# vkit-x/vkit

Measured on AMD Instinct MI355X. Metric: Mpixels/s (2048^2 RGB, geo+photo chain), higher is better.
Workload: dtype u8; 1 GPU; C3 fused chain: camera_cubic_curve remap (level 5) + gaussian_blur(sigma=1.0) + color_shift(37) + gaussion_noise(std=10.0, the numpy stream default_rng(5000 + i) drawn on the device inside every step), states built from the configs inside every step, 2048x2048x3 uint8, batch 256 per GPU; batch_per_gpu=256, image=2048x2048x3, noise_mode=tiles, states=built on the device from the configs inside every step (vkx_camera_states_dev), lanes=1

## Files before the change

### vkit_amd/csrc/fused.hip

```cpp
#include "vkx_internal.h"
#include "vkx_cell.h"
#include "vkx_color.h"

#include <float.h>
#include <memory>
#include <stdlib.h>
#include <string.h>

namespace {

constexpr int W = 64;
constexpr int RMAX = 3;
constexpr int NLDSCELL = 64;
#ifndef VKX_FUSED_NWAVES
#define VKX_FUSED_NWAVES 8
#endif
constexpr int NWAVES = VKX_FUSED_NWAVES;
constexpr int NTHREADS = 64 * NWAVES;
constexpr int ROWS_PER_WAVE = 8;
constexpr int WH = NWAVES * ROWS_PER_WAVE;
__host__ __device__ constexpr int tile_side(int R) { return (W - 2 * R) & ~3; }
__host__ __device__ constexpr int tile_height(int R) { return WH == W ? tile_side(R) : WH - 2 * R; }
#ifndef VKX_FUSED_CGROUP
#define VKX_FUSED_CGROUP 2
// ... 46 lines not shown
    int n;
};

struct TileRect {
    int x0, y0, x1, y1;
    __host__ __device__ bool empty() const { return x1 < x0 || y1 < y0; }
};
__host__ __device__ inline TileRect interior_rect(int dw, int dh, int R)
{
    const int Tw = tile_side(R), Th = tile_height(R);
    TileRect r;
    r.x0 = (R + Tw - 1) / Tw;
    r.y0 = (R + Th - 1) / Th;
    r.x1 = dw - W + R >= 0 ? (dw - W + R) / Tw : -1;
    r.y1 = dh - WH + R >= 0 ? (dh - WH + R) / Th : -1;
    return r;
}

struct TileBin {
    int rmin, cmin;
    int rmax1, cmax1;
};

struct CellR {
    int ex[4], edx[4];
    short vx[4], vy[4];
    int flags, pad;
};
static_assert(sizeof(CellR) == 56, "CellR mirrors the tail of CellC");

__device__ __forceinline__ int find_item(const int *__restrict__ prefix, int n, int v)
{
    int lo = 0, hi = n - 1;
    while (lo < hi) {
        const int mid = (lo + hi + 1) >> 1;
        if (prefix[mid] <= v) lo = mid; else hi = mid - 1;
    }
    return lo;
}

constexpr int kLocalBins = 1024;

__global__ void __launch_bounds__(256) k_chain_setup(const ItemDev *__restrict__ items, const int *__restrict__ cell_prefix,
                                                     int n_items, int total_cells, int slots,
                                                     vkc::CellC *__restrict__ cells, TileBin *__restrict__ bins,
                                                     int *__restrict__ deferred )
{
    __shared__ int lbins[kLocalBins * 4];
    __shared__ int s_item, s_tiles_x, s_ty_min, s_ty_max;
    const int gid = blockIdx.x * 256 + threadIdx.x;
    const bool active = gid < total_cells;
    int ii = -1, r = 0, c = 0, tx0 = 0, tx1 = -1, ty0 = 0, ty1 = -1, tiles_x = 1;
    if (active) {
        ii = find_item(cell_prefix, n_items, gid);
        const ItemDev &it = items[ii];
        const int cell = gid - it.cell_base;
        vkc::CellC rec;
        int xmin, xmax, ymin, ymax;
        if (vkc::build_cell<vkc::kCellDirectOnly>(it.sv, it.dv, it.rows, it.cols, cell, rec, xmin, xmax, ymin, ymax)) cells[gid] = rec;
        else deferred[1 + atomicAdd(&deferred[0], 1)] = gid;
        r = cell / (it.cols - 1); c = cell - r * (it.cols - 1);
        const int Tw = tile_side(it.R), Th = tile_height(it.R);
        tx0 = (xmin - it.R) / Tw; tx1 = (xmax + it.R) / Tw; ty0 = (ymin - it.R) / Th; ty1 = (ymax + it.R) / Th;
        if (xmin - it.R < 0) tx0 = 0;
        if (ymin - it.R < 0) ty0 = 0;
        tiles_x = it.tiles_x;
        tx1 = min(tx1, tiles_x - 1);
        ty1 = min(ty1, it.tiles_y - 1);
    }
    if (threadIdx.x == 0) { s_item = ii; s_tiles_x = tiles_x; s_ty_min = INT_MAX; s_ty_max = -1; }
    __syncthreads();
    const bool local = active && ii == s_item && ty0 <= ty1 && tx0 <= tx1;
    if (local) { atomicMin(&s_ty_min, ty0); atomicMax(&s_ty_max, ty1); }
    __syncthreads();
    const int tymin = s_ty_min, nb = s_ty_max >= tymin ? (s_ty_max - tymin + 1) * s_tiles_x : 0;
    const bool use_lds = nb > 0 && nb <= kLocalBins;
    if (use_lds)
        for (int i = threadIdx.x; i < nb; i += 256) {
            lbins[4 * i] = 0x7f7f7f7f; lbins[4 * i + 1] = 0x7f7f7f7f; lbins[4 * i + 2] = 0; lbins[4 * i + 3] = 0;
        }
    __syncthreads();
    for (int ty = ty0; ty <= ty1; ty++)
        for (int tx = tx0; tx <= tx1; tx++) {
            if (local && use_lds) {
                int *b = lbins + 4 * ((ty - tymin) * tiles_x + tx);
                atomicMin(b, r); atomicMin(b + 1, c); atomicMax(b + 2, r + 1); atomicMax(b + 3, c + 1);
            } else {
                TileBin *b = bins + (size_t)ii * slots + ty * tiles_x + tx;
                atomicMin(&b->rmin, r);
                atomicMin(&b->cmin, c);
                atomicMax(&b->rmax1, r + 1);
                atomicMax(&b->cmax1, c + 1);
            }
        }
    __syncthreads();
    if (use_lds)
        for (int i = threadIdx.x; i < nb; i += 256) {
            if (lbins[4 * i + 2] == 0) continue;
            TileBin *b = bins + (size_t)s_item * slots + tymin * s_tiles_x + i;
            atomicMin(&b->rmin, lbins[4 * i]);
            atomicMin(&b->cmin, lbins[4 * i + 1]);
            atomicMax(&b->rmax1, lbins[4 * i + 2]);
            atomicMax(&b->cmax1, lbins[4 * i + 3]);
        }
}

__global__ void __launch_bounds__(64) k_chain_setup_svd(const ItemDev *__restrict__ items, const int *__restrict__ cell_prefix,
                                                        int n_items, vkc::CellC *__restrict__ cells,
                                                        const int *__restrict__ deferred)
{
    const int n = deferred[0];
    const int sub = threadIdx.x & 7;
    for (int j = blockIdx.x * 8 + (threadIdx.x >> 3); j < n; j += gridDim.x * 8) {
        const int gid = deferred[1 + j];
        const ItemDev &it = items[find_item(cell_prefix, n_items, gid)];
        vkc::CellC rec;
        int xmin, xmax, ymin, ymax;
        vkc::build_cell<vkc::kCellJacobiGroup8>(it.sv, it.dv, it.rows, it.cols, gid - it.cell_base, rec, xmin, xmax, ymin, ymax);
        if (sub == 0) cells[gid] = rec;
    }
}

__device__ __forceinline__ int div_small(int n, int d, float rcp_d)
{
    int q = (int)(((float)n + 0.5f) * rcp_d);
    const int r = n - q * d;
    q += r >= d ? 1 : 0;
    q -= r < 0 ? 1 : 0;
    return q;
}

__device__ __forceinline__ uint32_t mad_u24(uint32_t a, uint32_t b, uint32_t c)
{
    uint32_t r;
    asm("v_mad_u32_u24 %0, %1, %2, %3" : "=v"(r) : "v"(a), "v"(b), "v"(c));
    return r;
}

__device__ __forceinline__ uint32_t mad_u24_ks(uint32_t k_uniform, uint32_t b, uint32_t c)
{
    return __umul24(k_uniform, b) + c;
}
__device__ __forceinline__ uint32_t mad_u24_cs(uint32_t a, uint32_t b, uint32_t c_uniform)
{
    return __umul24(a, b) + c_uniform;
}

typedef unsigned short ushort2_t __attribute__((ext_vector_type(2)));
__device__ __forceinline__ uint32_t dot2_u16_ks(uint32_t k_uniform, uint32_t b, uint32_t c)
{
    return __builtin_amdgcn_udot2(__builtin_bit_cast(ushort2_t, k_uniform), __builtin_bit_cast(ushort2_t, b), c, false);
}

__device__ __forceinline__ uint64_t uniform64(uint64_t v)
{
    const uint32_t lo = __builtin_amdgcn_readfirstlane((uint32_t)v), hi = __builtin_amdgcn_readfirstlane((uint32_t)(v >> 32));
    return ((uint64_t)hi << 32) | lo;
}

__device__ __forceinline__ void div_pair(double nx, double ny, double de, double &qx, double &qy)
{
    bool fdx, fdy, fnx, fny;
    const double sdx = __builtin_amdgcn_div_scale(nx, de, false, &fdx);
    const double sdy = __builtin_amdgcn_div_scale(ny, de, false, &fdy);
    if (__builtin_amdgcn_ballot_w64(__double_as_longlong(sdx) != __double_as_longlong(sdy)) != 0) {
        qx = nx / de;
        qy = ny / de;
        return;
    }
    double r = __builtin_amdgcn_rcp(sdx);
    double e = fma(-sdx, r, 1.0);
    r = fma(r, e, r);
    e = fma(-sdx, r, 1.0);
    r = fma(r, e, r);
    const double snx = __builtin_amdgcn_div_scale(nx, de, true, &fnx);
    const double sny = __builtin_amdgcn_div_scale(ny, de, true, &fny);
    const double px = snx * r, py = sny * r;
    const double ex = fma(-sdx, px, snx), ey = fma(-sdx, py, sny);
    qx = __builtin_amdgcn_div_fixup(__builtin_amdgcn_div_fmas(ex, r, px, fnx), de, nx);
    qy = __builtin_amdgcn_div_fixup(__builtin_amdgcn_div_fmas(ey, r, py, fny), de, ny);
}

__device__ __forceinline__ bool div_pair_f32_fast(double nx, double ny, double de, float &fx, float &fy)
{
    double r = __builtin_amdgcn_rcp(de);
    double e = fma(-de, r, 1.0);
    r = fma(r, e, r);
    e = fma(-de, r, 1.0);
    r = fma(r, e, r);
    const double qx = nx * r, qy = ny * r;
    const uint32_t lx = (uint32_t)__double_as_longlong(qx) & 0x1fffffffu, ly = (uint32_t)__double_as_longlong(qy) & 0x1fffffffu;
    const bool danger = (lx - (0x10000000u - 16u)) < 32u || (ly - (0x10000000u - 16u)) < 32u;
    fx = (float)qx;
    fy = (float)qy;
    return __builtin_amdgcn_ballot_w64(danger) == 0;
}

__device__ __forceinline__ void rim_sample_rgb(gsrc_t src, int sh, int sw, ptrdiff_t sstride, int X, int Y, uint32_t &prb, uint32_t &pg)
{
    const int sx = vkd::sat_short(X >> 5), sy = vkd::sat_short(Y >> 5);
    const int fx = X & 31, fy = Y & 31;
    prb = 0; pg = 0;
    if (sx >= sw || sx + 1 < 0 || sy >= sh || sy + 1 < 0) return;
    const bool x0 = sx >= 0, x1 = sx + 1 < sw, y0 = sy >= 0, y1 = sy + 1 < sh;
    const gsrc_t r0 = src + (ptrdiff_t)sy * sstride + (ptrdiff_t)sx * 3, r1 = r0 + sstride;
    const int w00 = (32 - fy) * (32 - fx), w01 = (32 - fy) * fx, w10 = fy * (32 - fx), w11 = fy * fx;
    uint32_t c[3];
#pragma unroll
    for (int k = 0; k < 3; k++) {
        const int v0 = (x0 && y0) ? r0[k] : 0;
        const int v1 = (x1 && y0) ? r0[3 + k] : 0;
        const int v2 = (x0 && y1) ? r1[k] : 0;
        const int v3 = (x1 && y1) ? r1[3 + k] : 0;
        c[k] = (uint32_t)(v0 * w00 + v1 * w01 + v2 * w10 + v3 * w11 + 512) >> 10;
    }
    prb = c[0] | (c[2] << 16);
    pg = c[1];
}

struct HsvLut {
    int sdiv[256];
    int hdiv[256];
};

__device__ __forceinline__ void hue_shift_px(const int *sdiv, const int *hdiv, int delta, int &r, int &g, int &b)
{
    int H, S, V;
    vkd::rgb2hsv_full<true>(sdiv, hdiv, r, g, b, H, S, V);
    H = (H + delta) & 255;
    vkd::hsv2rgb_full(H, S, V, r, g, b);
}

constexpr int P_ = 97;
constexpr int kPairPitch = 2 * P_;
constexpr size_t kLdsOwn = sizeof(uint32_t) * WH * P_;
constexpr size_t kLdsHbB = 1024;
constexpr size_t kLdsCellR = sizeof(CellR) * NLDSCELL;
constexpr size_t kLdsCellH = sizeof(double) * 9 * NLDSCELL;
constexpr size_t kLdsLut = sizeof(int) * 512;
constexpr size_t kLdsSel = sizeof(uint32_t) * 8;
constexpr size_t kLdsNoiseRows = sizeof(uint32_t) * 2 * WH;
constexpr size_t kFusedLds = kLdsOwn + kLdsHbB + kLdsCellR + kLdsCellH + kLdsLut + kLdsSel + 16 + kLdsNoiseRows;

typedef const double __attribute__((address_space(3))) *lds_cdouble_t;


__device__ __forceinline__ int cvt_i32_sat(float v)
{
    int r;
    asm("v_cvt_i32_f32 %0, %1" : "=v"(r) : "v"(v));
    return r;
}

__device__ __forceinline__ uint32_t add_noise_u8x4(uint32_t px, uint32_t n01, uint32_t n23)
{
    typedef unsigned short pk16 __attribute__((ext_vector_type(2)));
    pk16 lo = __builtin_bit_cast(pk16, __builtin_amdgcn_perm(px, px, 0x0c010c00u));
    pk16 hi = __builtin_bit_cast(pk16, __builtin_amdgcn_perm(px, px, 0x0c030c02u));
    lo += __builtin_bit_cast(pk16, n01);
    hi += __builtin_bit_cast(pk16, n23);
    uint32_t lo8, hi8;
    asm("v_sat_pk_u8_i16 %0, %1" : "=v"(lo8) : "v"(__builtin_bit_cast(uint32_t, lo)));
    asm("v_sat_pk_u8_i16 %0, %1" : "=v"(hi8) : "v"(__builtin_bit_cast(uint32_t, hi)));
    return __builtin_amdgcn_perm(hi8, lo8, 0x05040100u);
}

template <int KIND, bool STREAK = false, int RC = -1>
__device__ __forceinline__ void chain_tile(const ItemDev &it, const int tx, const int ty,
                                           const vkc::CellC *__restrict__ cells, const TileBin &bin,
                                           const HsvLut *__restrict__ lut, int phase_limit, const ElemPack *els = nullptr)
{
    constexpr bool INTERIOR = KIND == 1, EMPTY = KIND == 2;
    extern __shared__ __attribute__((aligned(16))) unsigned char smem[];
    uint32_t *own = (uint32_t *)smem;
    uint16_t *hbB = (uint16_t *)(smem + kLdsOwn);
    CellR *lcr = (CellR *)(smem + kLdsOwn + kLdsHbB);
    double *lch = (double *)(smem + kLdsOwn + kLdsHbB + kLdsCellR);
    int *lsdiv = (int *)(smem + kLdsOwn + kLdsHbB + kLdsCellR + kLdsCellH);
    int *lhdiv = lsdiv + 256;
    uint32_t *lsel = (uint32_t *)(lhdiv + 256);
    int *lflag = (int *)(lsel + 8);
    uint32_t *lnrow = (uint32_t *)(smem + kLdsOwn + kLdsHbB + kLdsCellR + kLdsCellH + kLdsLut + kLdsSel + 16);

    const int tid = threadIdx.x, lane = tid & 63, wave = __builtin_amdgcn_readfirstlane(tid >> 6);
    const int R = RC >= 0 ? RC : it.R, K = 2 * R + 1, Tw = tile_side(R), Th = tile_height(R);
    const int dw = it.dw, dh = it.dh;
    const int x0 = tx * Tw, y0 = ty * Th;
    const int tw = INTERIOR ? Tw : min(Tw, dw - x0), th = INTERIOR ? Th : min(Th, dh - y0);
    const int wx0 = x0 - R, wy0 = y0 - R;
    const int cx0 = INTERIOR ? wx0 : max(wx0, 0), cx1 = INTERIOR ? wx0 + W : min(wx0 + W, dw);
    const int cy0 = INTERIOR ? wy0 : max(wy0, 0), cy1 = INTERIOR ? wy0 + WH : min(wy0 + WH, dh);

    const gsrc_t src = (gsrc_t)it.src;
    const ptrdiff_t sstride = it.sstride;
    const int sh = it.sh, sw = it.sw;

    const int ocx = lane - R;
    const bool ocol = ocx >= 0 && ocx < tw;
    const int r0 = bin.rmin, c0 = bin.cmin;
    const int nr = max(0, bin.rmax1 - bin.rmin), ncol = max(0, bin.cmax1 - bin.cmin);
    const int nc = bin.rmax1 > 0 ? nr * ncol : 0;
    const int cw = it.cols - 1;
    const vkc::CellC *gcell = cells + it.cell_base;

    constexpr int kRecPerLane = NLDSCELL / (NTHREADS / 16);
    static_assert(NLDSCELL == kRecPerLane * (NTHREADS / 16), "whole records per lane and chunk");
    const float rcp_ncol = __builtin_amdgcn_rcpf((float)max(ncol, 1));
    auto chunk_fetch = [&](int base, int cn_, unsigned long long (&v)[kRecPerLane]) {
#pragma unroll
        for (int h = 0; h < kRecPerLane; h++) {
            const int rec = (tid >> 4) + h * (NTHREADS / 16);
            v[h] = 0;
            if (rec < cn_) {
                const int k = base + rec;
                const int rr = div_small(k, ncol, rcp_ncol), cc = k - rr * ncol;
                const unsigned long long VKX_GLOBAL *s8 =
                    (const unsigned long long VKX_GLOBAL *)(gcell + (r0 + rr) * cw + (c0 + cc));
                v[h] = s8[tid & 15];
            }
        }
    };
    auto chunk_store = [&](int cn_, const unsigned long long (&v)[kRecPerLane]) {
#pragma unroll
        for (int h = 0; h < kRecPerLane; h++) {
            const int rec = (tid >> 4) + h * (NTHREADS / 16), part = tid & 15;
            if (rec < cn_) {
                if (part < 8) ((unsigned long long *)(lch + rec * 9))[part] = v[h];
                else if (part < 15) ((unsigned long long *)(lcr + rec))[part - 8] = v[h];
            }
        }
    };
    auto load_chunk = [&](int base, int cn_) {
        unsigned long long v[kRecPerLane];
        chunk_fetch(base, cn_, v);
        chunk_store(cn_, v);
    };

    typedef uint32_t u32x2 __attribute__((ext_vector_type(2)));
    u32x2 nrec = {0u, 0u};
    const bool nrows_here = !(KIND == 3) && wave < WH / 64 && it.noise_rows != nullptr;
    const int nrow_y = wave * 64 + lane;
    if (nrows_here && nrow_y < th)
        nrec = ((const u32x2 VKX_GLOBAL *)it.noise_rows)[(size_t)(y0 + nrow_y) * (size_t)it.tiles_x + (size_t)tx];

    uint32_t kq[2 * RMAX + 1];
#pragma unroll
    for (int i = 0; i < 2 * RMAX + 1; i++) kq[i] = (R > 0 && i < K) ? it.kq[i < K - 1 - i ? i : K - 1 - i] : 0;
    if constexpr (!EMPTY) {
        unsigned long long first[kRecPerLane];
        chunk_fetch(0, min(NLDSCELL, nc), first);
        int lutv = 0;
        uint32_t selv = 0;
        if (it.hue_on) {
            if (NTHREADS == 512 || tid < 512) lutv = tid < 256 ? lut->sdiv[tid] : lut->hdiv[tid - 256];
            if (tid < 8) selv = vkd::kHsvSelectors[tid];
        }
#pragma unroll
        for (int i = 0; i < (WH * P_ / 4 + NTHREADS - 1) / NTHREADS; i++)
            if (tid + i * NTHREADS < WH * P_ / 4) ((uint4 *)own)[tid + i * NTHREADS] = make_uint4(0, 0, 0, 0);
        if (it.hue_on) {
            if (NTHREADS == 512 || tid < 512) lsdiv[tid] = lutv;
            if (tid < 8) lsel[tid] = selv;
        }
        if (tid == 0) *lflag = 0;
        if (nrows_here) *(u32x2 *)(lnrow + 2 * nrow_y) = nrec;
        for (int base = 0; base < (INTERIOR ? 1 : max(nc, 1)); base += NLDSCELL) {
            const int cn_ = INTERIOR ? nc : min(NLDSCELL, nc - base);
            if (base > 0) {
                __syncthreads();
                load_chunk(base, cn_);
            } else {
                chunk_store(cn_, first);
            }
            __syncthreads();
            if (phase_limit == 11) return;
            int *lpref = (int *)hbB;
            int *lylo = lpref + NLDSCELL + 1;
            if (wave == 0) {
                int hk = 0, ylo = 0;
                bool flagged = false;
                if (lane < cn_) {
                    const CellR &c = lcr[lane];
                    flagged = c.flags & 1;
                    int vmin = INT_MAX, vmax = INT_MIN;
#pragma unroll
                    for (int i = 0; i < 4; i++) { vmin = min(vmin, (int)c.vy[i]); vmax = max(vmax, (int)c.vy[i]); }
                    ylo = max(vmin, cy0);
                    hk = max(0, min(vmax, cy1) - ylo);
                }
                int incl = hk;
#pragma unroll
                for (int d = 1; d < 64; d <<= 1) {
                    const int t = __shfl_up(incl, d, 64);
                    if (lane >= d) incl += t;
                }
                lpref[lane + 1] = incl;
                if (lane == 0) lpref[0] = 0;
                lylo[lane] = ylo;
                if (__builtin_amdgcn_ballot_w64(flagged) != 0 && lane == 0) *lflag = 1;
            }
            __syncthreads();
            if (phase_limit == 12) return;
            const int nrows = lpref[NLDSCELL];
            for (int p = tid; p < nrows; p += NTHREADS) {
                int lo = 0, hi = cn_ - 1;
                while (lo < hi) {
                    const int mid = (lo + hi + 1) >> 1;
                    if (lpref[mid] <= p) lo = mid; else hi = mid - 1;
                }
                const int kk = lo;
                const int y = lylo[kk] + (p - lpref[kk]);
                const int row = y - wy0;
                const CellR &c = lcr[kk];
                const uint32_t tag = (uint32_t)(base + kk) + 1;
                int xs[4], n = 0, xmin = INT_MAX, xmax = INT_MIN;
#pragma unroll
                for (int i = 0; i < 4; i++) {
                    const int a = (i + 3) & 3;
                    const int ya = c.vy[a], yb = c.vy[i];
                    xmin = min(xmin, (int)c.vx[i]);
                    xmax = max(xmax, (int)c.vx[i]);
                    const int e0 = min(ya, yb), e1 = max(ya, yb);
                    if (e0 != e1 && e0 <= y && y < e1) xs[n++] = c.ex[i] + (y - e0) * c.edx[i];
                }
                for (int a = 1; a < n; a++) {
                    const int v = xs[a];
                    int b = a - 1;
                    while (b >= 0 && xs[b] > v) { xs[b + 1] = xs[b]; b--; }
                    xs[b + 1] = v;
                }
                const bool check = c.flags & 1;
                const double h6 = check ? lch[kk * 9 + 6] : 0.0, h7 = check ? lch[kk * 9 + 7] : 0.0;
                uint32_t *o = own + row * P_ - wx0;
                for (int a = 0; a + 1 < n; a += 2) {
                    const int x1 = max(max((xs[a] + 65535) >> 16, xmin), cx0);
                    const int x2 = min(min(xs[a + 1] >> 16, xmax), cx1 - 1);
                    if (!check) {
                        uint32_t *q = o + x1;
                        int left = x2 - x1 + 1;
                        for (; left >= 4; left -= 4, q += 4) {
                            atomicMax(q, tag); atomicMax(q + 1, tag); atomicMax(q + 2, tag); atomicMax(q + 3, tag);
                        }
                        if (left >= 1) atomicMax(q, tag);
                        if (left >= 2) atomicMax(q + 1, tag);
                        if (left >= 3) atomicMax(q + 2, tag);
                    } else {
                        for (int x = x1; x <= x2; x++) {
                            if (fma(1.0, 1.0, fma(h7, (double)y, h6 * (double)x)) == 0) continue;
                            atomicMax(o + x, tag);
                        }
                    }
                }
            }
            if (phase_limit == 13) return;
            for (int p = NTHREADS - 1 - tid; p < cn_ * 4; p += NTHREADS) {
                const int kk = p >> 2, i = p & 3;
                const CellR &c = lcr[kk];
                const uint32_t tag = (uint32_t)(base + kk) + 1;
                const int a = (i + 3) & 3;
                int lx = c.vx[a], ly = c.vy[a], rx = c.vx[i], ry = c.vy[i];
                if (rx < lx) { const int t1 = lx, t2 = ly; lx = rx; ly = ry; rx = t1; ry = t2; }
                const int dx = rx - lx, dy = ry - ly, ady = dy < 0 ? -dy : dy, sy = dy < 0 ? -1 : 1;
                const bool ymajor = ady > dx;
                const int dmaj = ymajor ? ady : dx, dmin = ymajor ? dx : ady;
                int k0, k1;
                if (ymajor) {
                    if (sy > 0) { k0 = max(0, cy0 - ly); k1 = min(ady, cy1 - 1 - ly); }
                    else        { k0 = max(0, ly - (cy1 - 1)); k1 = min(ady, ly - cy0); }
                } else {
                    k0 = max(0, cx0 - lx); k1 = min(dx, cx1 - 1 - lx);
                }
                if (k0 > k1) continue;
                int m = 0;
                {
                    const int num = 2 * k0 * dmin - dmaj;
                    if (dmaj != 0 && num > 0) m = (int)(((uint32_t)num + 2u * (uint32_t)dmaj - 1u) / (2u * (uint32_t)dmaj));
                }
                int err = (int)((uint32_t)dmaj - 2u * (uint32_t)dmin * (uint32_t)(k0 + 1) + 2u * (uint32_t)dmaj * (uint32_t)m);
                const int up = 2 * dmaj - 2 * dmin, down = -2 * dmin;
                int px = (ymajor ? lx + m : lx + k0) - wx0, py = (ymajor ? ly + sy * k0 : ly + sy * m) - wy0;
                const int ax = ymajor ? 0 : 1, ay = ymajor ? sy : 0, bx = ymajor ? 1 : 0, by = ymajor ? 0 : sy;
                const int lox = cx0 - wx0, nx_ = cx1 - cx0, loy = cy0 - wy0, ny_ = cy1 - cy0;
                const bool check = c.flags & 1;
                if (!check) {
                    for (int s = k0; s <= k1; s++) {
                        const bool inside = INTERIOR ? ((unsigned)px < (unsigned)W && (unsigned)py < (unsigned)WH)
                                                     : ((unsigned)(px - lox) < (unsigned)nx_ && (unsigned)(py - loy) < (unsigned)ny_);
                        if (inside) atomicMax(own + py * P_ + px, tag);
                        const bool step = err < 0;
                        err += step ? up : down;
                        px += ax + (step ? bx : 0);
                        py += ay + (step ? by : 0);
                    }
                } else {
                    const double h6 = lch[kk * 9 + 6], h7 = lch[kk * 9 + 7];
                    for (int s = k0; s <= k1; s++) {
                        const bool inside = (unsigned)(px - lox) < (unsigned)nx_ && (unsigned)(py - loy) < (unsigned)ny_;
                        if (inside && !(fma(1.0, 1.0, fma(h7, (double)(py + wy0), h6 * (double)(px + wx0))) == 0))
                            atomicMax(own + py * P_ + px, tag);
                        const bool step = err < 0;
                        err += step ? up : down;
                        px += ax + (step ? bx : 0);
                        py += ay + (step ? by : 0);
                    }
                }
            }
        }
        __syncthreads();
        if (phase_limit == 1) return;

        if (!INTERIOR && nc > NLDSCELL) {
            load_chunk(0, NLDSCELL);
            __syncthreads();
        }

        const int gx = wx0 + lane;
        const bool colok = INTERIOR || (gx >= cx0 && gx < cx1);
        int srcl[2 * RMAX + 1];
#pragma unroll
        for (int i = 0; i < 2 * RMAX + 1; i++) {
            int s = (R > 0 && i < K) ? (INTERIOR ? lane + i - R : vkd::reflect101(gx + i - R, dw) - wx0) : lane;
            srcl[i] = min(max(s, 0), W - 1) << 2;
        }
        const unsigned fast_xlim = (unsigned)max(sw - 2, 0), fast_ylim = (unsigned)max(sh - 1, 0);
        const double fxd = (double)gx;
        const bool exact_div = __builtin_amdgcn_readfirstlane(*lflag) != 0;
        for (int g0 = 0; g0 < ROWS_PER_WAVE; g0 += CGROUP) {
            int X[CGROUP], Y[CGROUP];
            bool rowok[CGROUP];
#pragma unroll
            for (int u = 0; u < CGROUP; u++) {
                const int ly = wave * ROWS_PER_WAVE + g0 + u;
                const int gy = wy0 + ly;
                rowok[u] = INTERIOR || (gy >= cy0 && gy < cy1);
                X[u] = 0; Y[u] = 0;
                if (rowok[u] && colok) {
                    const uint32_t o = own[ly * P_ + lane];
                    if (o != 0) {
                        const int k = (int)o - 1;
                        double h[8];
                        if (INTERIOR || k < NLDSCELL) {
                            lds_cdouble_t hp = (lds_cdouble_t)(lch + __umul24(k, 9));
                            asm volatile("" : "+v"(hp));
#pragma unroll
                            for (int j = 0; j < 8; j++) h[j] = hp[j];
                        } else {
                            const vkc::CellC VKX_GLOBAL *gc =
                                (const vkc::CellC VKX_GLOBAL *)(gcell + (r0 + div_small(k, ncol, rcp_ncol)) * cw + (c0 + k - div_small(k, ncol, rcp_ncol) * ncol));
#pragma unroll
                            for (int j = 0; j < 8; j++) h[j] = gc->H[j];
                        }
                        const double fy = (double)gy;
                        const double nx = fma(h[2], 1.0, fma(h[1], fy, h[0] * fxd));
                        const double ny = fma(h[5], 1.0, fma(h[4], fy, h[3] * fxd));
                        const double de = fma(1.0, 1.0, fma(h[7], fy, h[6] * fxd));
                        float qxf, qyf;
                        if (exact_div || !div_pair_f32_fast(nx, ny, de, qxf, qyf)) {
                            double qx, qy;
                            div_pair(nx, ny, de, qx, qy);
                            X[u] = vkd::cv_round((float)qx * 32.f);
                            Y[u] = vkd::cv_round((float)qy * 32.f);
                        } else {
                            X[u] = cvt_i32_sat(rintf(qxf * 32.f));
                            Y[u] = cvt_i32_sat(rintf(qyf * 32.f));
                        }
                    }
                }
            }
            if constexpr (KIND == 3) {
#pragma unroll
                for (int u = 0; u < CGROUP; u++) {
                    const int gy = wy0 + wave * ROWS_PER_WAVE + g0 + u;
                    if (!(rowok[u] && colok)) continue;
                    const int sx = X[u] >> 5, sy = Y[u] >> 5, fx = X[u] & 31, fy = Y[u] & 31;
                    const bool inner = (unsigned)sx < fast_xlim && (unsigned)sy < fast_ylim;
                    const int w00 = (32 - fy) * (32 - fx), w01 = (32 - fy) * fx, w10 = fy * (32 - fx), w11 = fy * fx;
                    for (int e = 0; e < els->n; e++) {
                        const ItemDev::Elem el = els->el[e];
                        if (el.is_f32) {
                            float v;
                            if (inner) {
                                typedef float f32x2_u4 __attribute__((ext_vector_type(2), aligned(4)));
                                const float VKX_GLOBAL *q0 = (const float VKX_GLOBAL *)el.src + (ptrdiff_t)sy * el.sstride + sx;
                                const f32x2_u4 a = *(const f32x2_u4 VKX_GLOBAL *)q0, b = *(const f32x2_u4 VKX_GLOBAL *)(q0 + el.sstride);
                                const float ax = fx * (1.f / 32), ay = fy * (1.f / 32), bx = 1.f - ax, by = 1.f - ay;
                                const float p0 = a.x * (by * bx), p1 = a.y * (by * ax), p2 = b.x * (ay * bx), p3 = b.y * (ay * ax);
                                v = ((p0 + p1) + p2) + p3;
                            } else {
                                v = vkd::sample_f32((const float VKX_GLOBAL *)el.src, sh, sw, el.sstride, X[u], Y[u]);
                            }
                            ((float VKX_GLOBAL *)el.dst)[(ptrdiff_t)gy * el.dstride + gx] = v;
                        } else {
                            gdst_t d = (gdst_t)el.dst + (ptrdiff_t)gy * el.dstride + (ptrdiff_t)gx * el.cn;
                            const gsrc_t sp = (gsrc_t)el.src;
                            if (el.cn == 1) {
                                if (inner) {
                                    const gsrc_t q0 = sp + (ptrdiff_t)sy * el.sstride + sx;
                                    const uint32_t a = *(const u16_u1 VKX_GLOBAL *)q0, b = *(const u16_u1 VKX_GLOBAL *)(q0 + el.sstride);
                                    d[0] = (uint8_t)(((a & 0xff) * w00 + (a >> 8) * w01 + (b & 0xff) * w10 + (b >> 8) * w11 + 512) >> 10);
                                } else {
                                    { uint8_t p1[1]; vkd::sample_u8<1>(sp, sh, sw, el.sstride, X[u], Y[u], p1); d[0] = p1[0]; }
                                }
                            } else if (el.cn == 3) {
                                uint8_t p3[3];
                                if (inner) {
                                    const gsrc_t q0 = sp + (ptrdiff_t)sy * el.sstride + (ptrdiff_t)sx * 3;
                                    const unsigned long long a = *(const u64_u1 VKX_GLOBAL *)q0, b = *(const u64_u1 VKX_GLOBAL *)(q0 + el.sstride);
#pragma unroll
                                    for (int k = 0; k < 3; k++) {
                                        const int v0 = (int)((a >> (8 * k)) & 0xff), v1 = (int)((a >> (8 * (k + 3))) & 0xff);
                                        const int v2 = (int)((b >> (8 * k)) & 0xff), v3 = (int)((b >> (8 * (k + 3))) & 0xff);
                                        p3[k] = (uint8_t)((v0 * w00 + v1 * w01 + v2 * w10 + v3 * w11 + 512) >> 10);
                                    }
                                } else {
                                    vkd::sample_u8<3>(sp, sh, sw, el.sstride, X[u], Y[u], p3);
                                }
                                d[0] = p3[0]; d[1] = p3[1]; d[2] = p3[2];
                            } else {
                                uint8_t p4[4];
                                if (inner) {
                                    const gsrc_t q0 = sp + (ptrdiff_t)sy * el.sstride + (ptrdiff_t)sx * 4;
                                    const unsigned long long a = *(const u64_u1 VKX_GLOBAL *)q0, b = *(const u64_u1 VKX_GLOBAL *)(q0 + el.sstride);
#pragma unroll
                                    for (int k = 0; k < 4; k++) {
                                        const int v0 = (int)((a >> (8 * k)) & 0xff), v1 = (int)((a >> (8 * (k + 4))) & 0xff);
                                        const int v2 = (int)((b >> (8 * k)) & 0xff), v3 = (int)((b >> (8 * (k + 4))) & 0xff);
                                        p4[k] = (uint8_t)((v0 * w00 + v1 * w01 + v2 * w10 + v3 * w11 + 512) >> 10);
                                    }
                                } else {
                                    vkd::sample_u8<4>(sp, sh, sw, el.sstride, X[u], Y[u], p4);
                                }
                                *(u32_u1 VKX_GLOBAL *)d = (uint32_t)p4[0] | ((uint32_t)p4[1] << 8) | ((uint32_t)p4[2] << 16) |
                                                 ((uint32_t)p4[3] << 24);
                            }
                        }
                    }
                }
                continue;
            }
            unsigned long long ta[CGROUP], tb[CGROUP];
            bool fast[CGROUP];
#pragma unroll
            for (int u = 0; u < CGROUP; u++) {
                const int sx = X[u] >> 5, sy = Y[u] >> 5;
                fast[u] = rowok[u] && colok && (unsigned)sx < fast_xlim && (unsigned)sy < fast_ylim;
                ta[u] = 0; tb[u] = 0;
                if (fast[u]) {
                    const uint32_t o0 = __umul24((uint32_t)sy, (uint32_t)sstride) + __umul24((uint32_t)sx, 3u);
                    ta[u] = *(const u64_u1 VKX_GLOBAL *)(src + (size_t)o0);
                    tb[u] = *(const u64_u1 VKX_GLOBAL *)(src + (size_t)(o0 + (uint32_t)sstride));
                }
            }
            uint32_t prb[CGROUP], pg[CGROUP];
#pragma unroll
            for (int u = 0; u < CGROUP; u++) {
                prb[u] = 0; pg[u] = 0;
                if (!rowok[u]) continue;
                if (colok) {
                    const int fx = X[u] & 31, fy = Y[u] & 31;
                    if (fast[u]) {
                        const uint32_t wx = (uint32_t)(32 - fx) | ((uint32_t)fx << 24);
                        const uint32_t t0 = (uint32_t)ta[u], t1 = (uint32_t)(ta[u] >> 32), b0 = (uint32_t)tb[u], b1 = (uint32_t)(tb[u] >> 32);
                        const uint32_t ar = __builtin_amdgcn_udot4(t0, wx, 0u, false);
                        const uint32_t ag = __builtin_amdgcn_udot4(__builtin_amdgcn_alignbyte(t1, t0, 1), wx, 0u, false);
                        const uint32_t ab = __builtin_amdgcn_udot4(__builtin_amdgcn_alignbyte(t1, t0, 2), wx, 0u, false);
                        const uint32_t br = __builtin_amdgcn_udot4(b0, wx, 0u, false);
                        const uint32_t bg = __builtin_amdgcn_udot4(__builtin_amdgcn_alignbyte(b1, b0, 1), wx, 0u, false);
                        const uint32_t bb = __builtin_amdgcn_udot4(__builtin_amdgcn_alignbyte(b1, b0, 2), wx, 0u, false);
                        const uint32_t wy0 = (uint32_t)(32 - fy), wy1 = (uint32_t)fy;
                        const uint32_t r = mad_u24(br, wy1, mad_u24_cs(ar, wy0, 512u)) >> 10;
                        const uint32_t g = mad_u24(bg, wy1, mad_u24_cs(ag, wy0, 512u)) >> 10;
                        const uint32_t b = mad_u24(bb, wy1, mad_u24_cs(ab, wy0, 512u)) >> 10;
                        prb[u] = r | (b << 16);
                        pg[u] = g;
                    } else {
                        rim_sample_rgb(src, sh, sw, sstride, X[u], Y[u], prb[u], pg[u]);
                    }
                }
            }
            static_assert(CGROUP == 2, "phase D works on the window-row pair of one iteration");
            const int ly0 = wave * ROWS_PER_WAVE + g0;
            if (!(rowok[0] || rowok[1])) continue;
            if (R > 0) {
                const uint32_t gg = pg[0] | (pg[1] << 16);
                uint32_t a0 = 0, a1 = 0, ag = 0;
#pragma unroll
                for (int i = 0; i < 2 * RMAX + 1; i++) {
                    if (i < K) {
                        uint32_t v0 = prb[0], v1 = prb[1], vg = gg;
                        if (!(INTERIOR && RC >= 0 && i == RC)) {
                            v0 = (uint32_t)__builtin_amdgcn_ds_bpermute(srcl[i], (int)prb[0]);
                            v1 = (uint32_t)__builtin_amdgcn_ds_bpermute(srcl[i], (int)prb[1]);
                            vg = (uint32_t)__builtin_amdgcn_ds_bpermute(srcl[i], (int)gg);
                        }
                        a0 = mad_u24_ks(kq[i], v0, a0);
                        a1 = mad_u24_ks(kq[i], v1, a1);
                        ag = mad_u24_ks(kq[i], vg, ag);
                    }
                }
                uint32_t *pl = own + ly0 * P_ + lane;
                pl[0] = __builtin_amdgcn_perm(a1, a0, 0x05040100u);
                pl[64] = ag;
                pl[128] = __builtin_amdgcn_perm(a1, a0, 0x07060302u);
            } else {
#pragma unroll
                for (int u = 0; u < CGROUP; u++)
                    if (rowok[u]) own[(ly0 + u) * P_ + lane] = (prb[u] & 0xffu) | (pg[u] << 8) | (prb[u] & 0xff0000u);
            }
        }
        if constexpr (KIND == 3) return;
        __syncthreads();
        if (phase_limit == 2) return;

    }

    const ItemDev VKX_GLOBAL *ite_ = (const ItemDev VKX_GLOBAL *)&it;
    asm volatile("" : "+s"(ite_));
    const ItemDev VKX_GLOBAL &ite = *ite_;
    const gdst_t dst = (gdst_t)uniform64((uint64_t)ite.dst);
    const int16_t VKX_GLOBAL *noise = (const int16_t VKX_GLOBAL *)uniform64((uint64_t)ite.noise);
    const ptrdiff_t dstride = (ptrdiff_t)uniform64((uint64_t)ite.dstride), nstride = (ptrdiff_t)uniform64((uint64_t)ite.nstride);
    uint32_t nzA[ROWS_PER_WAVE];
    uint32_t nzB[ROWS_PER_WAVE];
    const bool tiled = noise && __builtin_amdgcn_readfirstlane(ite.noise_tiled) != 0;
    if constexpr (EMPTY) {
        if (nrows_here) *(u32x2 *)(lnrow + 2 * nrow_y) = nrec;
        if (tiled) __syncthreads();
    }
    const int full4 = (tw >> 2) << 2;
    const bool grouped = !STREAK && (INTERIOR || ocx < full4);
    const uint32_t g4 = (uint32_t)((ocx >> 2) * 12 + (ocx & 3) * 4);
    const uint32_t k3 = grouped ? g4 : (uint32_t)(ocx * 3);
    const bool nlane = ocol && !(grouped && (ocx & 3) == 3);
    u32x2 nrow = {0u, 0u};
    if (tiled) nrow = *(const u32x2 *)(lnrow + 2 * (wave + NWAVES * (lane & 7)));
#pragma unroll
    for (int i = 0; i < ROWS_PER_WAVE; i++) {
        nzA[i] = 0; nzB[i] = 0;
        const int cy = wave + NWAVES * i;
        if (noise && nlane && cy < th) {
            const int16_t VKX_GLOBAL *np_;
            if (tiled) {
                const int16_t VKX_GLOBAL *rowp = noise + (size_t)(uint32_t)__builtin_amdgcn_readlane((int)nrow.x, i);
                const uint32_t sd = (uint32_t)__builtin_amdgcn_readlane((int)nrow.y, i);
                uint32_t off = k3;
                if ((sd & 0xffffu) < 3u * W) {
                    asm volatile("" ::: "memory");
                    off += k3 >= (sd & 0xffffu) ? (uint32_t)((int)sd >> 16) : 0u;
                }
                np_ = rowp + off;
            } else {
                np_ = noise + (ptrdiff_t)(y0 + cy) * nstride + (ptrdiff_t)x0 * 3 + (ptrdiff_t)k3;
            }
            if (grouped) {
                const unsigned long long v = *(const u64_u1 VKX_GLOBAL *)np_;
                nzA[i] = (uint32_t)v;
                nzB[i] = (uint32_t)(v >> 32);
            } else {
                nzA[i] = *(const u32_u1 VKX_GLOBAL *)np_;
                nzB[i] = *(const u16_u1 VKX_GLOBAL *)(np_ + 2);
            }
        }
    }
    uint32_t wpair[RMAX + 1];
#pragma unroll
    for (int q = 0; q <= RMAX; q++) {
        const uint32_t e0 = 2 * q < K ? kq[2 * q < 2 * RMAX + 1 ? 2 * q : 0] : 0u, e1 = 2 * q + 1 < K ? kq[2 * q + 1 < 2 * RMAX + 1 ? 2 * q + 1 : 0] : 0u;
        const uint32_t o0 = (q > 0 && 2 * q - 1 < K) ? kq[q > 0 ? 2 * q - 1 : 0] : 0u, o1 = 2 * q < K ? kq[2 * q < 2 * RMAX + 1 ? 2 * q : 0] : 0u;
        wpair[q] = (wave & 1) ? (o0 | (o1 << 16)) : (e0 | (e1 << 16));
    }
    const bool hue_on = __builtin_amdgcn_readfirstlane(ite.hue_on) != 0;
    const int hue_delta = __builtin_amdgcn_readfirstlane(ite.hue_delta);
    const int right4 = min(lane + 1, 63) << 2;
    const uint32_t dcol4 = (uint32_t)(x0 * 3) + g4;
    const bool streak_on = STREAK && ite.streak_on != 0;
    const int sxm = streak_on ? (x0 + ocx) % ite.streak_step : 0;
    const int sxd = streak_on ? (x0 + ocx) % ite.streak_dash_step : 0;
    uint32_t epx = 0;
    if constexpr (EMPTY) {
        int er = src[0], eg = src[1], eb = src[2];
        if (hue_on) hue_shift_px(lut->sdiv, lut->hdiv, hue_delta, er, eg, eb);
        epx = (uint32_t)er | ((uint32_t)eg << 8) | ((uint32_t)eb << 16);
    }
#pragma unroll
    for (int i = 0; i < ROWS_PER_WAVE; i++) {
        const int cy = wave + NWAVES * i;
        if (cy >= th) continue;
        const int gy = y0 + cy;
        uint32_t P = epx;
        if constexpr (!EMPTY) {
            if (R > 0) {
                int r, g, b;
                if constexpr (INTERIOR && RC > 0) {
                    const uint32_t *pl = own + (cy & ~1) * P_ + lane;
                    uint32_t ar = 32768u, ag = 32768u, ab = 32768u;
#pragma unroll
                    for (int q = 0; q <= RC; q++) {
                        ar = dot2_u16_ks(wpair[q], pl[q * kPairPitch], ar);
                        ag = dot2_u16_ks(wpair[q], pl[q * kPairPitch + 64], ag);
                        ab = dot2_u16_ks(wpair[q], pl[q * kPairPitch + 128], ab);
                    }
                    r = (int)(ar >> 16); g = (int)(ag >> 16); b = (int)(ab >> 16);
                } else {
                    uint32_t a0 = 0, a1 = 0, a2 = 0;
#pragma unroll
                    for (int j = 0; j < 2 * RMAX + 1; j++) {
                        if (j < K) {
                            const int yy = INTERIOR ? cy + j : vkd::reflect101(gy + j - R, dh) - wy0;
                            const uint16_t *h16 = (const uint16_t *)(own + (yy & ~1) * P_ + lane) + (yy & 1);
                            a0 += __umul24(kq[j], (uint32_t)h16[0]);
                            a1 += __umul24(kq[j], (uint32_t)h16[128]);
                            a2 += __umul24(kq[j], (uint32_t)h16[256]);
                        }
                    }
                    r = (int)((a0 + 32768u) >> 16); g = (int)((a1 + 32768u) >> 16); b = (int)((a2 + 32768u) >> 16);
                }
                if (phase_limit == 20) {
                    const int yy = INTERIOR ? cy + R : vkd::reflect101(gy, dh) - wy0;
                    const uint16_t *h16 = (const uint16_t *)(own + (yy & ~1) * P_ + lane) + (yy & 1);
                    r = h16[0] >> 8; g = h16[128] >> 8; b = h16[256] >> 8;
                }
                if (hue_on) P = vkd::hue_shift_packed(lsdiv, lhdiv, lsel, hue_delta, r, g, b);
                else P = (uint32_t)r | ((uint32_t)g << 8) | ((uint32_t)b << 16);
            } else {
                P = own[(cy + R) * P_ + lane];
                if (hue_on) P = vkd::hue_shift_packed(lsdiv, lhdiv, lsel, hue_delta, (int)(P & 0xff), (int)((P >> 8) & 0xff),
                                                      (int)((P >> 16) & 0xff));
            }
        }
        if ((STREAK || !INTERIOR) && ((noise && !grouped) || (STREAK && streak_on))) {
            int r = (int)(P & 0xff), g = (int)((P >> 8) & 0xff), b = (int)((P >> 16) & 0xff);
            if (noise) {
                r = vkd::clamp_u8((int)(int16_t)(r + (int)(nzA[i] & 0xffff)));
                g = vkd::clamp_u8((int)(int16_t)(g + (int)(nzA[i] >> 16)));
                b = vkd::clamp_u8((int)(int16_t)(b + (int)(nzB[i] & 0xffff)));
            }
            if (STREAK && streak_on) {
                const int ym = gy % ite.streak_step, yd = gy % ite.streak_dash_step;
                bool mv = ite.streak_vert && sxm < ite.streak_thickness;
                bool mh = ite.streak_hori && ym < ite.streak_thickness;
                if (ite.streak_dash) {
                    if (yd < ite.streak_dash_gap) mv = false;
                    if (sxd < ite.streak_dash_gap) mh = false;
                }
                const float w1 = ite.streak_alpha, w0 = 1.0f - w1;
                int *ch[3] = {&r, &g, &b};
#pragma unroll
                for (int c = 0; c < 3; c++) {
                    int v = *ch[c];
                    const int col = ite.streak_color[c];
                    if (mv) { const float t0 = w0 * (float)v, t1 = w1 * (float)col; v = ite.streak_copy ? col : (int)(uint8_t)(t0 + t1); }
                    if (mh) { const float t0 = w0 * (float)v, t1 = w1 * (float)col; v = ite.streak_copy ? col : (int)(uint8_t)(t0 + t1); }
                    *ch[c] = v;
                }
            }
            P = (uint32_t)r | ((uint32_t)g << 8) | ((uint32_t)b << 16);
        }
        const uint32_t Pn = (uint32_t)__builtin_amdgcn_ds_bpermute(right4, (int)P);
        gdst_t drow = dst + (ptrdiff_t)gy * dstride + (ptrdiff_t)x0 * 3;
        if (ocol) {
            const int m = ocx & 3;
            if (INTERIOR || ocx < full4) {
                if (m < 3) {
                    uint32_t wv = (P >> (8 * m)) | (Pn << (24 - 8 * m));
                    if (!STREAK && noise) wv = add_noise_u8x4(wv, nzA[i], nzB[i]);
                    const uint32_t off = (uint32_t)gy * (uint32_t)dstride + dcol4;
                    *(u32_u1 VKX_GLOBAL *)(dst + (size_t)off) = wv;
                }
            } else {
                gdst_t d = drow + ocx * 3;
                d[0] = (uint8_t)P; d[1] = (uint8_t)(P >> 8); d[2] = (uint8_t)(P >> 16);
            }
        }
    }
}

template <bool STREAK>
__global__ void __launch_bounds__(NTHREADS, VKX_FUSED_WAVES_PER_EU) k_chain_fused(const ItemDev *__restrict__ items,
                                                          const vkc::CellC *__restrict__ cells,
                                                          const TileBin *__restrict__ bins, int bin_slots,
                                                          int *__restrict__ over_count, int2 *__restrict__ over_list, int over_slots,
                                                          const HsvLut *__restrict__ lut, int phase_limit)
{
    const ItemDev &it = items[blockIdx.y];
    const int rw = it.rect_w;
    const int nrect = rw * it.rect_h;
    const int per = (nrect + 7) >> 3;
    const int run = (int)((blockIdx.x + blockIdx.y) & 7), pos = (int)(blockIdx.x >> 3);
    const int rl = run * per + pos;
    if (pos >= per || rl >= nrect) return;
    if (phase_limit == 10) return;
    const int ry = __builtin_amdgcn_readfirstlane(div_small(rl, rw, __builtin_amdgcn_rcpf((float)rw)));
    const int tx = it.rect_x0 + rl - ry * rw, ty = it.rect_y0 + ry;
    const int tl = ty * it.tiles_x + tx;
    const TileBin bin = bins[(size_t)blockIdx.y * bin_slots + tl];
    const int nc = bin.rmax1 > 0 ? max(0, bin.rmax1 - bin.rmin) * max(0, bin.cmax1 - bin.cmin) : 0;
#ifdef VKX_FUSED_CENSUS
    (void)nc;
    chain_tile<1, STREAK, VKX_FUSED_CENSUS>(it, tx, ty, cells, bin, lut, phase_limit);
    return;
#endif
    if (nc == 0) chain_tile<2, STREAK>(it, tx, ty, cells, bin, lut, phase_limit);
    else if (nc <= NLDSCELL && phase_limit != 3) {
        switch (it.R) {
        case 0: chain_tile<1, STREAK, 0>(it, tx, ty, cells, bin, lut, phase_limit); break;
        case 1: chain_tile<1, STREAK, 1>(it, tx, ty, cells, bin, lut, phase_limit); break;
        case 2: chain_tile<1, STREAK, 2>(it, tx, ty, cells, bin, lut, phase_limit); break;
        default: chain_tile<1, STREAK, 3>(it, tx, ty, cells, bin, lut, phase_limit); break;
        }
    } else if (threadIdx.x == 0) {
        const int k = atomicAdd(over_count, 1);
        if (k < over_slots) over_list[k] = make_int2((int)blockIdx.y, tl);
    }
}

template <bool STREAK>
__global__ void __launch_bounds__(NTHREADS, VKX_FUSED_WAVES_PER_EU) k_chain_fused_rim(const ItemDev *__restrict__ items,
                                                          const vkc::CellC *__restrict__ cells,
                                                          const TileBin *__restrict__ bins, int bin_slots,
                                                          const HsvLut *__restrict__ lut, int phase_limit)
{
    if (phase_limit == 10) return;
    const ItemDev &it = items[blockIdx.y];
    const int tiles_x = it.tiles_x, rw = it.rect_w, rh = it.rect_h;
    const int nrim = tiles_x * it.tiles_y - rw * rh;
    const int per = (nrim + 7) >> 3;
    const int run = (int)((blockIdx.x + blockIdx.y) & 7), pos = (int)(blockIdx.x >> 3);
    const int q = run * per + pos;
    if (pos >= per || q >= nrim) return;
    int tl;
    const int top = it.rect_y0 * tiles_x, bottom = (it.tiles_y - it.rect_y0 - rh) * tiles_x;
    if (rw * rh == 0 || q < top) tl = q;
    else if (q < top + bottom) tl = q - top + (it.rect_y0 + rh) * tiles_x;
    else {
        const int m = q - top - bottom, side = tiles_x - rw;
        const int r = __builtin_amdgcn_readfirstlane(div_small(m, side, __builtin_amdgcn_rcpf((float)side)));
        const int c = m - r * side;
        tl = (it.rect_y0 + r) * tiles_x + (c < it.rect_x0 ? c : c + rw);
    }
    const TileBin bin = bins[(size_t)blockIdx.y * bin_slots + tl];
    const int ty = __builtin_amdgcn_readfirstlane(div_small(tl, tiles_x, __builtin_amdgcn_rcpf((float)tiles_x)));
    const int tx = tl - ty * tiles_x;
    const int nc = bin.rmax1 > 0 ? max(0, bin.rmax1 - bin.rmin) * max(0, bin.cmax1 - bin.cmin) : 0;
    if (nc == 0) chain_tile<2, STREAK>(it, tx, ty, cells, bin, lut, phase_limit);
    else {
        switch (it.R) {
        case 0: chain_tile<0, STREAK, 0>(it, tx, ty, cells, bin, lut, phase_limit); break;
        case 1: chain_tile<0, STREAK, 1>(it, tx, ty, cells, bin, lut, phase_limit); break;
        case 2: chain_tile<0, STREAK, 2>(it, tx, ty, cells, bin, lut, phase_limit); break;
        default: chain_tile<0, STREAK, 3>(it, tx, ty, cells, bin, lut, phase_limit); break;
        }
    }
}

constexpr int kOverGrid = 512;
template <bool STREAK>
__global__ void __launch_bounds__(NTHREADS, 4) k_chain_fused_over(const ItemDev *__restrict__ items,
                                                          const vkc::CellC *__restrict__ cells,
                                                          const TileBin *__restrict__ bins, int bin_slots,
                                                          const int *__restrict__ over_count, const int2 *__restrict__ over_list,
                                                          int over_slots, const HsvLut *__restrict__ lut, int phase_limit)
{
    const int n_over = min(*over_count, over_slots);
    if ((int)blockIdx.x >= n_over || phase_limit == 10) return;
    for (int k = (int)blockIdx.x; k < n_over; k += (int)gridDim.x) {
// ... 438 lines not shown
```

### vkit_amd/csrc/vkx_color.h

```cpp
#ifndef VKX_COLOR_H_
#define VKX_COLOR_H_

#include "vkx_internal.h"

namespace vkd {

template <bool WRAP_H = false>
__device__ __forceinline__ void rgb2hsv_full(const int *sdiv, const int *hdiv, int r, int g, int b, int &H, int &S, int &V)
{
    const int v = max(b, max(g, r)), vmin = min(b, min(g, r));
    const int diff = v - vmin;
    const int vr = v == r ? -1 : 0, vg = v == g ? -1 : 0;
    S = (__mul24(diff, sdiv[v]) + (1 << 11)) >> 12;
    int hh = (vr & (g - b)) + (~vr & ((vg & (b - r + 2 * diff)) + ((~vg) & (r - g + 4 * diff))));
    hh = __mul24(hh, hdiv[diff]) + (1 << 11);
    hh >>= 12;
    if (!WRAP_H) hh += hh < 0 ? 256 : 0;
    H = hh;
    V = v;
}

__device__ __forceinline__ void hsv2rgb_full(int H, int S, int V, int &r, int &g, int &b)
{
    const float s = S * (1.0f / 255.0f);
    const float fv = V * (1.0f / 255.0f);
    const int h6 = __mul24(H, 6);
    const int sector = h6 >> 8;
    const float h = (float)(h6 & 255) * (1.0f / 256);
    const bool odd = sector & 1;
    const int rot = sector >> 1;
    const float t0 = fv;
    const float t1 = fv * (1.f - s);
    const float tt = fv * (1.f - s * (odd ? h : 1.f - h));
    const float u0 = t1, u1 = odd ? t0 : tt, u2 = odd ? tt : t0;
    const float fb = rot == 0 ? u0 : (rot == 1 ? u1 : u2);
    const float fg = rot == 0 ? u1 : (rot == 1 ? u2 : u0);
    const float fr = rot == 0 ? u2 : (rot == 1 ? u0 : u1);
    r = __float2int_rn(fr * 255.0f);
    g = __float2int_rn(fg * 255.0f);
    b = __float2int_rn(fb * 255.0f);
}

__device__ constexpr uint32_t kHsvSelectors[8] = {0x0c040001u, 0x0c040100u, 0x0c000104u, 0x0c010004u,
                                                  0x0c010400u, 0x0c000401u, 0x0c0c0c0cu, 0x0c0c0c0cu};

__device__ __forceinline__ uint32_t hue_shift_packed(const int *sdiv, const int *hdiv, const uint32_t *sel, int delta,
                                                     int r, int g, int b)
{
    int H, S, V;
    rgb2hsv_full<true>(sdiv, hdiv, r, g, b, H, S, V);
    const uint32_t h6 = __umul24((uint32_t)(H + delta) & 255u, 6u);
    const float s = (float)S * (1.0f / 255.0f);
    const float fv = (float)V * (1.0f / 255.0f);
    const float h = (float)(h6 & 255u) * (1.0f / 256);
    const float x = (h6 & 256u) ? h : 1.f - h;
    const float t1 = fv * (1.f - s);
    const float tt = fv * (1.f - s * x);
    const float m1 = t1 * 255.0f + 12582912.0f;
    const float mt = tt * 255.0f + 12582912.0f;
    const uint32_t lo = __float_as_uint(mt) | ((uint32_t)V << 8);
    return __builtin_amdgcn_perm(__float_as_uint(m1), lo, sel[h6 >> 8]);
}

}

#endif
```

Measured before the change: 72140 Mpixels/s.

## Exploit symmetric blur taps with DPP shifts and packed u16 MADs

```diff
diff --git a/vkit_amd/csrc/fused.hip b/vkit_amd/csrc/fused.hip
--- a/vkit_amd/csrc/fused.hip
+++ b/vkit_amd/csrc/fused.hip
@@ -222,6 +222,20 @@
     return __builtin_amdgcn_udot2(__builtin_bit_cast(ushort2_t, k_uniform), __builtin_bit_cast(ushort2_t, b), c, false);
 }
 
+__device__ __forceinline__ uint32_t wave_shr1(uint32_t v)
+{
+    return (uint32_t)__builtin_amdgcn_mov_dpp((int)v, 0x138 , 0xf, 0xf, true);
+}
+__device__ __forceinline__ uint32_t wave_shl1(uint32_t v)
+{
+    return (uint32_t)__builtin_amdgcn_mov_dpp((int)v, 0x130 , 0xf, 0xf, true);
+}
+__device__ __forceinline__ uint32_t pk_mad_u16_ks(uint32_t k2_uniform, uint32_t b, uint32_t c)
+{
+    const ushort2_t k = __builtin_bit_cast(ushort2_t, k2_uniform);
+    return __builtin_bit_cast(uint32_t, (ushort2_t)(k * __builtin_bit_cast(ushort2_t, b) + __builtin_bit_cast(ushort2_t, c)));
+}
+
 __device__ __forceinline__ uint64_t uniform64(uint64_t v)
 {
     const uint32_t lo = __builtin_amdgcn_readfirstlane((uint32_t)v), hi = __builtin_amdgcn_readfirstlane((uint32_t)(v >> 32));
@@ -414,8 +428,23 @@
         nrec = ((const u32x2 VKX_GLOBAL *)it.noise_rows)[(size_t)(y0 + nrow_y) * (size_t)it.tiles_x + (size_t)tx];
 
     uint32_t kq[2 * RMAX + 1];
-#pragma unroll
-    for (int i = 0; i < 2 * RMAX + 1; i++) kq[i] = (R > 0 && i < K) ? it.kq[i < K - 1 - i ? i : K - 1 - i] : 0;
+    if constexpr (RC >= 0) {
+        uint32_t kh[RMAX + 1];
+#pragma unroll
+        for (int j = 0; j <= RMAX; j++) {
+            kh[j] = 0;
+            if (RC > 0 && j <= RC) {
+                kh[j] = (uint32_t)__builtin_amdgcn_readfirstlane((int)((uint32_t)it.kq[j] * 0x10001u));
+            }
+        }
+#pragma unroll
+        for (int i = 0; i < 2 * RMAX + 1; i++) kq[i] = i < K ? kh[i < K ? min(i, K - 1 - i) : 0] : 0;
+    } else {
+#pragma unroll
+        for (int i = 0; i < 2 * RMAX + 1; i++) kq[i] = (R > 0 && i < K) ? (uint32_t)it.kq[i < K - 1 - i ? i : K - 1 - i] * 0x10001u : 0;
+    }
+    const uint32_t kqc = RC >= 0 ? kq[RC >= 0 ? RC : 0] : (uint32_t)it.kq[R] * 0x10001u;
+    auto kw = [&](int i) { return kq[i] & 0xffffu; };
     if constexpr (!EMPTY) {
         unsigned long long first[kRecPerLane];
         chunk_fetch(0, min(NLDSCELL, nc), first);
@@ -586,12 +615,17 @@
 
         const int gx = wx0 + lane;
         const bool colok = INTERIOR || (gx >= cx0 && gx < cx1);
-        int srcl[2 * RMAX + 1];
-#pragma unroll
-        for (int i = 0; i < 2 * RMAX + 1; i++) {
-            int s = (R > 0 && i < K) ? (INTERIOR ? lane + i - R : vkd::reflect101(gx + i - R, dw) - wx0) : lane;
-            srcl[i] = min(max(s, 0), W - 1) << 2;
-        }
+        auto tap_lane = [&](int t) {
+            const int s = INTERIOR ? lane + t - R : vkd::reflect101(gx + t - R, dw) - wx0;
+            return min(max(s, 0), W - 1) << 2;
+        };
+        int srcl[RMAX], srcm[RMAX];
+#pragma unroll
+        for (int j = 0; j < RMAX; j++) {
+            srcl[j] = j < R ? tap_lane(j) : lane << 2;
+            srcm[j] = j < R ? tap_lane(K - 1 - j) : lane << 2;
+        }
+        const int srcc = tap_lane(R);
         const unsigned fast_xlim = (unsigned)max(sw - 2, 0), fast_ylim = (unsigned)max(sh - 1, 0);
         const double fxd = (double)gx;
         const bool exact_div = __builtin_amdgcn_readfirstlane(*lflag) != 0;
@@ -753,19 +787,39 @@
             if (!(rowok[0] || rowok[1])) continue;
             if (R > 0) {
                 const uint32_t gg = pg[0] | (pg[1] << 16);
-                uint32_t a0 = 0, a1 = 0, ag = 0;
-#pragma unroll
-                for (int i = 0; i < 2 * RMAX + 1; i++) {
-                    if (i < K) {
-                        uint32_t v0 = prb[0], v1 = prb[1], vg = gg;
-                        if (!(INTERIOR && RC >= 0 && i == RC)) {
-                            v0 = (uint32_t)__builtin_amdgcn_ds_bpermute(srcl[i], (int)prb[0]);
-                            v1 = (uint32_t)__builtin_amdgcn_ds_bpermute(srcl[i], (int)prb[1]);
-                            vg = (uint32_t)__builtin_amdgcn_ds_bpermute(srcl[i], (int)gg);
+                uint32_t c0 = prb[0], c1 = prb[1], cg = gg;
+                if (!INTERIOR) {
+                    c0 = (uint32_t)__builtin_amdgcn_ds_bpermute(srcc, (int)prb[0]);
+                    c1 = (uint32_t)__builtin_amdgcn_ds_bpermute(srcc, (int)prb[1]);
+                    cg = (uint32_t)__builtin_amdgcn_ds_bpermute(srcc, (int)gg);
+                }
+                uint32_t a0 = pk_mad_u16_ks(kqc, c0, 0u), a1 = pk_mad_u16_ks(kqc, c1, 0u), ag = pk_mad_u16_ks(kqc, cg, 0u);
+                if constexpr (INTERIOR) {
+                    uint32_t l0 = prb[0], l1 = prb[1], lg = gg, r0_ = prb[0], r1_ = prb[1], rg = gg;
+#pragma unroll
+                    for (int d = 1; d <= RMAX; d++) {
+                        if (d <= R) {
+                            l0 = wave_shr1(l0); l1 = wave_shr1(l1); lg = wave_shr1(lg);
+                            r0_ = wave_shl1(r0_); r1_ = wave_shl1(r1_); rg = wave_shl1(rg);
+                            a0 = pk_mad_u16_ks(kq[d <= R ? R - d : 0], l0 + r0_, a0);
+                            a1 = pk_mad_u16_ks(kq[d <= R ? R - d : 0], l1 + r1_, a1);
+                            ag = pk_mad_u16_ks(kq[d <= R ? R - d : 0], lg + rg, ag);
                         }
-                        a0 = mad_u24_ks(kq[i], v0, a0);
-                        a1 = mad_u24_ks(kq[i], v1, a1);
-                        ag = mad_u24_ks(kq[i], vg, ag);
+                    }
+                } else {
+#pragma unroll
+                    for (int j = 0; j < RMAX; j++) {
+                        if (j < R) {
+                            const uint32_t s0 = (uint32_t)__builtin_amdgcn_ds_bpermute(srcl[j], (int)prb[0]) +
+                                                (uint32_t)__builtin_amdgcn_ds_bpermute(srcm[j], (int)prb[0]);
+                            const uint32_t s1 = (uint32_t)__builtin_amdgcn_ds_bpermute(srcl[j], (int)prb[1]) +
+                                                (uint32_t)__builtin_amdgcn_ds_bpermute(srcm[j], (int)prb[1]);
+                            const uint32_t sg = (uint32_t)__builtin_amdgcn_ds_bpermute(srcl[j], (int)gg) +
+                                                (uint32_t)__builtin_amdgcn_ds_bpermute(srcm[j], (int)gg);
+                            a0 = pk_mad_u16_ks(kq[j], s0, a0);
+                            a1 = pk_mad_u16_ks(kq[j], s1, a1);
+                            ag = pk_mad_u16_ks(kq[j], sg, ag);
+                        }
                     }
                 }
                 uint32_t *pl = own + ly0 * P_ + lane;
@@ -833,10 +887,15 @@
         }
     }
     uint32_t wpair[RMAX + 1];
+    uint32_t ke[RMAX + 1];
+#pragma unroll
+    for (int j = 0; j <= RMAX; j++)
+        ke[j] = (INTERIOR && RC > 0 && j <= RC) ? (uint32_t)__builtin_amdgcn_readfirstlane((int)ite.kq[j]) : 0u;
+    auto kv = [&](int i) { return (INTERIOR && RC > 0) ? ke[i < K ? min(i, K - 1 - i) : 0] : kw(i); };
 #pragma unroll
     for (int q = 0; q <= RMAX; q++) {
-        const uint32_t e0 = 2 * q < K ? kq[2 * q < 2 * RMAX + 1 ? 2 * q : 0] : 0u, e1 = 2 * q + 1 < K ? kq[2 * q + 1 < 2 * RMAX + 1 ? 2 * q + 1 : 0] : 0u;
-        const uint32_t o0 = (q > 0 && 2 * q - 1 < K) ? kq[q > 0 ? 2 * q - 1 : 0] : 0u, o1 = 2 * q < K ? kq[2 * q < 2 * RMAX + 1 ? 2 * q : 0] : 0u;
+        const uint32_t e0 = 2 * q < K ? kv(2 * q < 2 * RMAX + 1 ? 2 * q : 0) : 0u, e1 = 2 * q + 1 < K ? kv(2 * q + 1 < 2 * RMAX + 1 ? 2 * q + 1 : 0) : 0u;
+        const uint32_t o0 = (q > 0 && 2 * q - 1 < K) ? kv(q > 0 ? 2 * q - 1 : 0) : 0u, o1 = 2 * q < K ? kv(2 * q < 2 * RMAX + 1 ? 2 * q : 0) : 0u;
         wpair[q] = (wave & 1) ? (o0 | (o1 << 16)) : (e0 | (e1 << 16));
     }
     const bool hue_on = __builtin_amdgcn_readfirstlane(ite.hue_on) != 0;
@@ -878,9 +937,9 @@
                         if (j < K) {
                             const int yy = INTERIOR ? cy + j : vkd::reflect101(gy + j - R, dh) - wy0;
                             const uint16_t *h16 = (const uint16_t *)(own + (yy & ~1) * P_ + lane) + (yy & 1);
-                            a0 += __umul24(kq[j], (uint32_t)h16[0]);
-                            a1 += __umul24(kq[j], (uint32_t)h16[128]);
-                            a2 += __umul24(kq[j], (uint32_t)h16[256]);
+                            a0 += __umul24(kw(j), (uint32_t)h16[0]);
+                            a1 += __umul24(kw(j), (uint32_t)h16[128]);
+                            a2 += __umul24(kw(j), (uint32_t)h16[256]);
                         }
                     }
                     r = (int)((a0 + 32768u) >> 16); g = (int)((a1 + 32768u) >> 16); b = (int)((a2 + 32768u) >> 16);
diff --git a/vkit_amd/csrc/vkx_color.h b/vkit_amd/csrc/vkx_color.h
--- a/vkit_amd/csrc/vkx_color.h
+++ b/vkit_amd/csrc/vkx_color.h
@@ -13,7 +13,7 @@
     const int vr = v == r ? -1 : 0, vg = v == g ? -1 : 0;
     S = (__mul24(diff, sdiv[v]) + (1 << 11)) >> 12;
     int hh = (vr & (g - b)) + (~vr & ((vg & (b - r + 2 * diff)) + ((~vg) & (r - g + 4 * diff))));
-    hh = __mul24(hh, hdiv[diff]) + (1 << 11);
+    asm("v_mad_i32_i24 %0, %1, %2, %3" : "=v"(hh) : "v"(hh), "v"(hdiv[diff]), "v"(1 << 11));
     hh >>= 12;
     if (!WRAP_H) hh += hh < 0 ? 256 : 0;
     H = hh;
```

Measured after the change: 72750 Mpixels/s, median of 6. No clear change (+0.9%).
